# tencent-ailab/V-Express

Hardware: AMD Instinct MI355X
Metric: decoded frames/sec at 512x512, 25 DDIM steps (higher is better)
Workload: dtype bf16; 1 GPU; 512x512, 16 frames (1 window(s) of 16, overlap 4), 25 DDIM steps, CFG 3.5, random-init UNet3D + ReferenceNet banks + sd-vae-ft-mse decode; frames=16, windows=1, parallelism=window x CFG-half units over 1 GPU(s)

## Files before the change

### v-express_amd/csrc/vx_gemm.hip

```cpp
#include "vx_common.h"
#include "vx_gemm_common.h"
#include "../../include/vexpress_hip.h"

#include <stdio.h>
#include <stdlib.h>
#include <string.h>

namespace {

#ifdef VX_GEMM_ABLATE
#define ABL(bit) (((VX_GEMM_ABLATE) & (bit)) != 0)
#else
#define ABL(bit) false
#endif

struct RowInfo {
  int pix_base;
  int iy0, ix0;
};

template <typename T>
__device__ __forceinline__ T sel3(int i, T a, T b, T c) { return i == 0 ? a : (i == 1 ? b : c); }

__device__ __attribute__((aligned(16))) const uint4 g_zero16 = {0u, 0u, 0u, 0u};

template <int N>
__device__ __forceinline__ void wait_vmcnt() {
  asm volatile("s_waitcnt vmcnt(%0)" ::"n"(N) : "memory");
}

typedef int i32x8_t __attribute__((ext_vector_type(8)));
__device__ __forceinline__ f32x4_t mfma16_f8(const uint4& a_lo, const uint4& a_hi, const uint4& b_lo, const uint4& b_hi,
                                             f32x4_t c) {
  const i32x8_t a = {(int)a_lo.x, (int)a_lo.y, (int)a_lo.z, (int)a_lo.w, (int)a_hi.x, (int)a_hi.y, (int)a_hi.z, (int)a_hi.w};
  const i32x8_t b = {(int)b_lo.x, (int)b_lo.y, (int)b_lo.z, (int)b_lo.w, (int)b_hi.x, (int)b_hi.y, (int)b_hi.z, (int)b_hi.w};
  return __builtin_amdgcn_mfma_scale_f32_16x16x128_f8f6f4(a, b, c, 0, 0, 0, 0x7f7f7f7f, 0, 0x7f7f7f7f);
}

template <int BM, int BN, int WARPS_M, int WARPS_N, int STAGES, int EPI, bool FAST, bool F8 = false, bool LNF = false,
          bool GNS = false>
__global__ __launch_bounds__(64 * WARPS_M * WARPS_N, 2) void gemm_kernel(const vx_gemm_params p) {
  static_assert(!F8 || FAST, "fp8 operands use the FAST addressing only");
  static_assert(!GNS || (EPI == VX_EPI_STORE && !F8 && !LNF), "GroupNorm partial sums come from the plain STORE epilogue");
  static_assert(!LNF || (FAST && !F8), "a folded LayerNorm sits in front of a plain bf16 linear");
  constexpr int ES = F8 ? 1 : 2;
  constexpr int BKE = 128 / ES;
  constexpr int CE = 16 / ES;
  constexpr int NTHREADS = 64 * WARPS_M * WARPS_N;
  constexpr int RPP = NTHREADS / 8;
  constexpr int WM = BM / WARPS_M, WN = BN / WARPS_N;
  constexpr int MI = WM / 16, NI = WN / 16;
  constexpr int NJ = F8 ? (NI % 2 == 0 ? 2 : 1) : (NI <= 5 ? NI : NI / 2);
  constexpr int A_IT = BM / RPP, B_IT = BN / RPP;
  constexpr int G = A_IT + B_IT;
  constexpr int STAGE_BYTES = (BM + BN) * 128;
  static_assert(WM == 64, "every wave owns a 64-row slab");
  static_assert(BM % RPP == 0 && BN % RPP == 0, "tile rows must be a multiple of the staging pass");
  static_assert(NI % NJ == 0, "fragment grouping");
  static_assert(G * (STAGES - 2) < 64, "vmcnt is 6 bits");
  extern __shared__ __attribute__((aligned(16))) char smem[];

  const int tid = threadIdx.x;
  const int lane = tid & 63, wave = __builtin_amdgcn_readfirstlane(tid >> 6);
  const int wm = wave / WARPS_N, wn = wave % WARPS_N;
  const int n_tiles = (p.n + BN - 1) / BN;
  const int nsplit = (EPI == VX_EPI_STORE && p.splitk > 1) ? p.splitk : 1;
  const int lid0 = xcd_remap(blockIdx.x, gridDim.x);
  const int split = lid0 % nsplit, lid = lid0 / nsplit;
  const int tile_m = lid / n_tiles, tile_n = lid - tile_m * n_tiles;
  const int m0 = tile_m * BM, n0 = tile_n * BN;

  const bf16_t* __restrict__ A1 = (const bf16_t*)p.a;
  const bf16_t* __restrict__ A2 = (const bf16_t*)p.a2;
  const bf16_t* __restrict__ Wt = (const bf16_t*)p.w;
  const int cin = p.c1 + p.c2;
  const int c1 = p.c1;
  const int up = p.upsample;
  const int h_eff = p.h_in << up, w_eff = p.w_in << up;
  const int hw_out = p.h_out * p.w_out;
  const int w_in = p.w_in, kw = p.kw, kh = p.kh;
  const int lda1 = p.lda1, lda2 = p.lda2;
  const bf16_t* const zsrc = reinterpret_cast<const bf16_t*>(&g_zero16);

  const int r0 = tid >> 3;
  const int cc = (tid & 7) ^ ((r0 >> 1) & 7);
  uint32_t aoff1[A_IT], aoff2[A_IT], boff[B_IT];
  const int nk_total = (p.k + BKE - 1) / BKE;
  const int kt_begin = (int)((long)split * nk_total / nsplit), kt_end = (int)((long)(split + 1) * nk_total / nsplit);
  int s_kt = kt_begin, s_ci, s_kx, s_ky;
  {
    const int tap0 = (kt_begin * BKE) / cin;
    s_ci = kt_begin * BKE - tap0 * cin;
    s_ky = tap0 / kw;
    s_kx = tap0 - s_ky * kw;
  }
  RowInfo ri[A_IT];
  long wrow[B_IT];
// ... 153 lines not shown
#pragma unroll
        for (int i = 0; i < MI; ++i)
#pragma unroll
          for (int j = 0; j < NJ; ++j) {
            if (ABL(8)) {
              asm volatile("" ::"v"(bfr[j].x), "v"(af[i].x));
              continue;
            }
            acc[i][j0 + j] = mfma16(bfr[j], af[i], acc[i][j0 + j]);
          }
      }
    }
    }
    stage = stage + 1 == STAGES ? 0 : stage + 1;
    fill = fill + 1 == STAGES ? 0 : fill + 1;
  }

  const float* __restrict__ bias = p.bias;
  const int lrow = lane & 15, lq = lane >> 4;
  const int wrow0 = m0 + wm * WM, wcol0 = n0 + wn * WN;

  if constexpr (F8) {
    const float* __restrict__ asc = p.a_scale;
    const float* __restrict__ wsc = p.w_scale;
    float sa_[MI];
#pragma unroll
    for (int i = 0; i < MI; ++i) sa_[i] = asc[min(wrow0 + i * 16 + lrow, p.m - 1)];
#pragma unroll
    for (int j = 0; j < NI; ++j) {
      const float4 sw = *reinterpret_cast<const float4*>(wsc + min(wcol0 + j * 16 + lq * 4, p.n - 4));
#pragma unroll
      for (int i = 0; i < MI; ++i) {
        acc[i][j][0] *= sa_[i] * sw.x; acc[i][j][1] *= sa_[i] * sw.y;
        acc[i][j][2] *= sa_[i] * sw.z; acc[i][j][3] *= sa_[i] * sw.w;
      }
    }
  }

  if constexpr (LNF) {
    const float2* __restrict__ st = reinterpret_cast<const float2*>(p.ln_stats);
    const float* __restrict__ cs = p.ln_colsum;
#pragma unroll
    for (int i = 0; i < MI; ++i) {
      const float2 t = st[min(wrow0 + i * 16 + lrow, p.m - 1)];
#pragma unroll
      for (int j = 0; j < NI; ++j) {
        const float4 s4 = *reinterpret_cast<const float4*>(cs + min(wcol0 + j * 16 + lq * 4, p.n - 4));
        acc[i][j][0] = t.y * (acc[i][j][0] - t.x * s4.x); acc[i][j][1] = t.y * (acc[i][j][1] - t.x * s4.y);
        acc[i][j][2] = t.y * (acc[i][j][2] - t.x * s4.z); acc[i][j][3] = t.y * (acc[i][j][3] - t.x * s4.w);
      }
    }
  }

  if (EPI == VX_EPI_STORE && nsplit > 1) {
    float* ws = (float*)p.splitk_ws + (size_t)split * p.m * p.n;
#pragma unroll
    for (int i = 0; i < MI; ++i) {
      const int m = wrow0 + i * 16 + lrow;
#pragma unroll
      for (int j = 0; j < NI; ++j) {
        const int n = wcol0 + j * 16 + lq * 4;
        if (m < p.m && n < p.n)
          *reinterpret_cast<float4*>(ws + (size_t)m * p.n + n) =
              make_float4(acc[i][j][0], acc[i][j][1], acc[i][j][2], acc[i][j][3]);
      }
    }
    return;
  }
  if constexpr (EPI == VX_EPI_STORE) {
    const float* __restrict__ rowbias = p.rowbias;
    const bf16_t* __restrict__ resid = (const bf16_t*)p.residual;
    const bool do_silu = p.act == VX_ACT_SILU, do_gelu = p.act == VX_ACT_GELU;
    const bool out_is_f32 = p.out_f32 != 0;
    const float alpha = p.alpha;
    float gcs[GNS ? NI * 4 : 1], gcq[GNS ? NI * 4 : 1];
    if constexpr (GNS) {
#pragma unroll
      for (int c = 0; c < NI * 4; ++c) gcs[c] = gcq[c] = 0.f;
    }
#pragma unroll
    for (int j0 = 0; j0 < NI; j0 += NJ) {
      int ncol[NJ], nc[NJ];
      float4 bv[NJ];
#pragma unroll
      for (int j = 0; j < NJ; ++j) {
        ncol[j] = wcol0 + (j0 + j) * 16 + lq * 4;
        nc[j] = min(ncol[j], p.n - 4);
        bv[j] = make_float4(0.f, 0.f, 0.f, 0.f);
      }
      if (bias != nullptr && !ABL(2)) {
#pragma unroll
        for (int j = 0; j < NJ; ++j) bv[j] = *reinterpret_cast<const float4*>(bias + nc[j]);
      }
#pragma unroll
      for (int i = 0; i < MI; ++i) {
        const int m = wrow0 + i * 16 + lrow;
        const int mc = min(m, p.m - 1);
        uint2 rv[NJ];
        float4 rb[NJ];
#pragma unroll
        for (int j = 0; j < NJ; ++j) {
          rv[j] = make_uint2(0u, 0u);
          rb[j] = make_float4(0.f, 0.f, 0.f, 0.f);
        }
        if (resid != nullptr && !ABL(2)) {
          const bf16_t* rrow = resid + (size_t)mc * p.ldr;
#pragma unroll
          for (int j = 0; j < NJ; ++j) rv[j] = *reinterpret_cast<const uint2*>(rrow + nc[j]);
        }
        if (rowbias != nullptr && !ABL(2)) {
          const float* rbrow = rowbias + (size_t)(mc / p.rows_per_group) * p.rowbias_ld;
#pragma unroll
          for (int j = 0; j < NJ; ++j) rb[j] = *reinterpret_cast<const float4*>(rbrow + nc[j]);
        }
#pragma unroll
        for (int j = 0; j < NJ; ++j) {
          const f32x4_t a4 = acc[i][j0 + j];
          float v[4] = {a4[0] + bv[j].x + rb[j].x, a4[1] + bv[j].y + rb[j].y, a4[2] + bv[j].z + rb[j].z,
                        a4[3] + bv[j].w + rb[j].w};
          if (do_silu) {
#pragma unroll
            for (int e = 0; e < 4; ++e) v[e] = silu_f(v[e]);
          } else if (do_gelu) {
#pragma unroll
            for (int e = 0; e < 4; ++e) v[e] = gelu_f(v[e]);
          }
#pragma unroll
          for (int e = 0; e < 4; ++e) v[e] *= alpha;
          v[0] += e16_lo(rv[j].x); v[1] += e16_hi(rv[j].x);
          v[2] += e16_lo(rv[j].y); v[3] += e16_hi(rv[j].y);
          if constexpr (GNS) {
            const uint2 pk = make_uint2(pack_bf16x2(v[0], v[1]), pack_bf16x2(v[2], v[3]));
            *reinterpret_cast<uint2*>((bf16_t*)p.out + (size_t)m * p.ldc + ncol[j]) = pk;
            const float g[4] = {e16_lo(pk.x), e16_hi(pk.x),
                                e16_lo(pk.y), e16_hi(pk.y)};
#pragma unroll
            for (int e = 0; e < 4; ++e) {
              gcs[(j0 + j) * 4 + e] += g[e];
              gcq[(j0 + j) * 4 + e] = fmaf(g[e], g[e], gcq[(j0 + j) * 4 + e]);
            }
          } else if (ABL(1)) {
            asm volatile("" ::"v"(v[0]), "v"(v[1]), "v"(v[2]), "v"(v[3]));
          } else if (m < p.m && ncol[j] < p.n) {
            if (out_is_f32) {
              *reinterpret_cast<float4*>((float*)p.out + (size_t)m * p.ldc + ncol[j]) =
                  make_float4(v[0], v[1], v[2], v[3]);
            } else {
              *reinterpret_cast<uint2*>((bf16_t*)p.out + (size_t)m * p.ldc + ncol[j]) =
                  make_uint2(pack_bf16x2(v[0], v[1]), pack_bf16x2(v[2], v[3]));
            }
          }
        }
      }
    }
    if constexpr (GNS) {
#pragma unroll
      for (int c = 0; c < NI * 4; ++c) {
        gcs[c] = row16_sum(gcs[c]);
        gcq[c] = row16_sum(gcq[c]);
      }
      float2* scr = reinterpret_cast<float2*>(smem + STAGES * STAGE_BYTES) + wave * WN;
      if (lrow == 0) {
#pragma unroll
        for (int j = 0; j < NI; ++j)
#pragma unroll
          for (int e = 0; e < 4; ++e) scr[j * 16 + lq * 4 + e] = make_float2(gcs[j * 4 + e], gcq[j * 4 + e]);
      }
      asm volatile("s_waitcnt lgkmcnt(0)" ::: "memory");
      const int cg = p.n / p.gn_groups;
      if (lane < WN / cg) {
        float a = 0.f, b = 0.f;
        for (int c = 0; c < cg; ++c) {
          const float2 t = scr[lane * cg + c];
          a += t.x;
          b += t.y;
        }
        const int frame = wrow0 / p.gn_hw, slab = (wrow0 - frame * p.gn_hw) >> 6, slabs = p.gn_hw >> 6;
        const int g = wcol0 / cg + lane;
        reinterpret_cast<float2*>(p.gn_ws)[(size_t)(frame * slabs + slab) * p.gn_groups + g] = make_float2(a, b);
      }
    }
  } else if constexpr (EPI == VX_EPI_GEGLU) {
    static_assert(MI % 2 == 0, "GEGLU pairs row blocks");
// ... 106 lines not shown
        }
        __syncthreads();
      }
    }
  }
}

__global__ __launch_bounds__(256) void splitk_reduce_kernel(const vx_gemm_params p) {
  const int n4 = p.n >> 2;
  const long total = (long)p.m * n4;
  const float* __restrict__ ws = (const float*)p.splitk_ws;
  const size_t slab = (size_t)p.m * p.n;
  for (long idx = (long)blockIdx.x * 256 + threadIdx.x; idx < total; idx += (long)gridDim.x * 256) {
    const int m = (int)(idx / n4), n = (int)(idx - (long)m * n4) * 4;
    float4 a = *reinterpret_cast<const float4*>(ws + (size_t)m * p.n + n);
    for (int s = 1; s < p.splitk; ++s) {
      const float4 b = *reinterpret_cast<const float4*>(ws + s * slab + (size_t)m * p.n + n);
      a.x += b.x; a.y += b.y; a.z += b.z; a.w += b.w;
    }
    float v[4] = {a.x, a.y, a.z, a.w};
    if (p.bias != nullptr) {
      const float4 b = *reinterpret_cast<const float4*>(p.bias + n);
      v[0] += b.x; v[1] += b.y; v[2] += b.z; v[3] += b.w;
    }
    if (p.rowbias != nullptr) {
      const float4 b =
          *reinterpret_cast<const float4*>(p.rowbias + (size_t)(m / p.rows_per_group) * p.rowbias_ld + n);
      v[0] += b.x; v[1] += b.y; v[2] += b.z; v[3] += b.w;
    }
    if (p.act == VX_ACT_SILU) {
#pragma unroll
      for (int e = 0; e < 4; ++e) v[e] = silu_f(v[e]);
    } else if (p.act == VX_ACT_GELU) {
#pragma unroll
      for (int e = 0; e < 4; ++e) v[e] = gelu_f(v[e]);
    }
#pragma unroll
    for (int e = 0; e < 4; ++e) v[e] *= p.alpha;
    if (p.residual != nullptr) {
      const uint2 r2 = *reinterpret_cast<const uint2*>((const bf16_t*)p.residual + (size_t)m * p.ldr + n);
      v[0] += e16_lo(r2.x); v[1] += e16_hi(r2.x);
      v[2] += e16_lo(r2.y); v[3] += e16_hi(r2.y);
    }
    if (p.out_f32) {
      *reinterpret_cast<float4*>((float*)p.out + (size_t)m * p.ldc + n) = make_float4(v[0], v[1], v[2], v[3]);
    } else {
      *reinterpret_cast<uint2*>((bf16_t*)p.out + (size_t)m * p.ldc + n) =
          make_uint2(pack_bf16x2(v[0], v[1]), pack_bf16x2(v[2], v[3]));
    }
  }
}

template <int BM, int BN, int WARPS_M, int WARPS_N, int STAGES, int EPI, bool FAST, bool F8 = false, bool LNF = false,
          bool GNS = false>
int launch_impl(const vx_gemm_params& p, hipStream_t stream) {
  constexpr int stage_bytes = STAGES * (BM + BN) * 128;
  constexpr int epi_bytes = (EPI == VX_EPI_SPLIT) ? BN * (64 + 4) * 4 : 0;
  constexpr int gns_bytes = GNS ? WARPS_M * BN * 8 : 0;
  constexpr int smem = (stage_bytes > epi_bytes ? stage_bytes : epi_bytes) + gns_bytes;
  constexpr int nthreads = 64 * WARPS_M * WARPS_N;
  static bool attr_set = false;
  auto kern = gemm_kernel<BM, BN, WARPS_M, WARPS_N, STAGES, EPI, FAST, F8, LNF, GNS>;
  if (!attr_set) {
    hipError_t e = hipFuncSetAttribute((const void*)kern, hipFuncAttributeMaxDynamicSharedMemorySize, smem);
    if (e != hipSuccess) {
      vx_set_error("vx_gemm: hipFuncSetAttribute(%d B LDS) failed: %s", smem, hipGetErrorString(e));
      return VX_ERR_HIP;
    }
    attr_set = true;
  }
  const int nsplit = (EPI == VX_EPI_STORE && p.splitk > 1) ? p.splitk : 1;
  long tiles = (long)ceil_div(p.m, BM) * ceil_div(p.n, BN) * nsplit;
  static char sym[112] = "";
  if (!sym[0]) {
    auto b = [](bool v) { return v ? "true" : "false"; };
    snprintf(sym, sizeof(sym), "gemm_kernel<%d, %d, %d, %d, %d, %d, %s, %s, %s, %s>", BM, BN, WARPS_M, WARPS_N, STAGES, EPI,
             b(FAST), b(F8), b(LNF), b(GNS));
  }
  g_vx_last_kernel = sym;
  hipLaunchKernelGGL(kern, dim3((unsigned)tiles), dim3(nthreads), smem, stream, p);
  int rc = vx_check_launch("vx_gemm");
  if (rc != 0 || nsplit == 1) return rc;
  long work = ((long)p.m * (p.n >> 2) + 255) / 256;
  hipLaunchKernelGGL(splitk_reduce_kernel, dim3((unsigned)(work < 2048 ? work : 2048)), dim3(256), 0, stream, p);
  return vx_check_launch("vx_gemm(split-K reduce)");
}

bool fast_ok(const vx_gemm_params& p) { return vx_gemm_fast_ok(p); }
}
bool vx_gemm_fast_ok(const vx_gemm_params& p) {
  static int disabled = -1;
  if (disabled < 0) disabled = getenv("VX_GEMM_NOFAST") != nullptr;
  if (disabled) return false;
  const int cin = p.c1 + p.c2;
  const unsigned long long rows_in = (unsigned long long)p.nb * p.h_in * p.w_in;
  return p.pad == 0 && p.upsample == 0 && (cin % 64) == 0 && (p.c1 % 64) == 0 && (p.k % 64) == 0 &&
         rows_in * (unsigned long long)p.lda1 * 2ull < (1ull << 32) &&
         (p.c2 == 0 || rows_in * (unsigned long long)p.lda2 * 2ull < (1ull << 32)) &&
         (unsigned long long)p.n * p.k * 2ull < (1ull << 32) &&
         (p.h_out - 1) * p.stride + p.kh <= p.h_in && (p.w_out - 1) * p.stride + p.kw <= p.w_in;
}
namespace {

template <int BM, int BN, int WARPS_M, int WARPS_N, int STAGES, int EPI>
int launch(const vx_gemm_params& p, hipStream_t stream) {
  if (p.ln_stats != nullptr) {
    if (!fast_ok(p)) {
      vx_set_error("vx_gemm: a folded LayerNorm needs a plain linear (k %% 64 == 0, no padding / upsampling)");
      return VX_ERR_UNSUPPORTED;
    }
    return launch_impl<BM, BN, WARPS_M, WARPS_N, STAGES, EPI, true, false, true>(p, stream);
  }
  if (fast_ok(p)) return launch_impl<BM, BN, WARPS_M, WARPS_N, STAGES, EPI, true>(p, stream);
  return launch_impl<BM, BN, WARPS_M, WARPS_N, STAGES, EPI, false>(p, stream);
}

template <int BM, int BN, int WARPS_M, int WARPS_N, int STAGES>
int launch_gns(const vx_gemm_params& p, hipStream_t stream) {
  if (fast_ok(p)) return launch_impl<BM, BN, WARPS_M, WARPS_N, STAGES, VX_EPI_STORE, true, false, false, true>(p, stream);
  return launch_impl<BM, BN, WARPS_M, WARPS_N, STAGES, VX_EPI_STORE, false, false, false, true>(p, stream);
}

bool prefer160(int n) {
  int w160 = ceil_div(n, 160) * 160 - n, w128 = ceil_div(n, 128) * 128 - n;
  return w160 * 128 <= w128 * 160;
}

enum { CFG_AUTO = 0, CFG_BIG = 1, CFG_SMALL = 2 };
int forced_cfg() {
  static int v = -1;
  if (v < 0) {
    const char* e = getenv("VX_GEMM_TILE");
    v = CFG_AUTO;
    if (e && !strcmp(e, "big")) v = CFG_BIG;
    if (e && !strcmp(e, "small")) v = CFG_SMALL;
  }
  return v;
}
bool use_big(const vx_gemm_params& p) {
  if ((p.n % 320) != 0 || p.splitk > 1) return false;
  int f = forced_cfg();
  if (f == CFG_BIG) return true;
  if (f == CFG_SMALL) return false;
  long tiles = (long)ceil_div(p.m, 256) * (p.n / 320);
  return tiles >= 256;
}

bool use_small64(const vx_gemm_params& p) {
  static int on = -1;
  if (on < 0) {
    const char* e = getenv("VX_GEMM_SMALL64");
    on = !(e && !strcmp(e, "0"));
  }
  if (!on || !prefer160(p.n) || p.out_f32) return false;
  const long tiles128 = (long)ceil_div(p.m, 128) * ceil_div(p.n, 160) * (p.splitk > 1 ? p.splitk : 1);
  static long lim = -1;
  if (lim < 0) {
    const char* e = getenv("VX_GEMM_SMALL64_BELOW");
    lim = e ? atol(e) : 256;
  }
  return tiles128 < lim && fast_ok(p);
}

enum { T_256x32 = 0, T_BIG, T_SMALL64, T_128x160, T_128x128, T_128x320, T_256x256 };
bool use_256x256(const vx_gemm_params& p) {
  static int on = -1;
  if (on < 0) {
    const char* e = getenv("VX_GEMM_T256X256");
    on = !(e && !strcmp(e, "0"));
  }
  return on && (p.n % 256) == 0 && p.n <= 1024 && p.splitk <= 1 && !p.out_f32 && (long)ceil_div(p.m, 256) * (p.n / 256) >= 256;
}
bool use_128x320(const vx_gemm_params& p) {
// ... 2 lines not shown
    const char* e = getenv("VX_GEMM_T128X320");
    on = e && !strcmp(e, "1");
  }
  return on && (p.n % 320) == 0 && p.splitk <= 1 && !p.out_f32;
}
int store_tile(const vx_gemm_params& p, bool gn = false) {
  if (p.n <= 32) return T_256x32;
  if (gn && (p.n % 160) == 0) return use_small64(p) ? T_SMALL64 : T_128x160;
  if (use_big(p)) return T_BIG;
  if (use_small64(p)) return T_SMALL64;
  if (use_128x320(p)) return T_128x320;
  if (prefer160(p.n)) return T_128x160;
  if (use_256x256(p)) return T_256x256;
  return T_128x128;
}

}

extern "C" int vx_gemm_gn_slabs(const vx_gemm_params* pp) {
  const vx_gemm_params& p = *pp;
  if (p.epi != VX_EPI_STORE || p.a_fp8 || p.out_f32 || p.ln_stats != nullptr || p.row_stats_out != nullptr ||
      (p.splitk > 1 && p.ring_hint != 2) || p.w_group_rows != 0)
    return 0;
  if (p.gn_groups <= 0 || p.gn_hw <= 0 || p.n <= 0 || (p.n % p.gn_groups) != 0 || (p.m % p.gn_hw) != 0) return 0;
  if (vx_gemm_ring_eligible(p)) return vx_gemm_ring_gn_slabs(p);
  if (p.splitk > 1) return 0;
  const int cg = p.n / p.gn_groups;
  const int tile = store_tile(p, true);
  if (tile != T_SMALL64 && tile != T_128x160) return 0;
  static int st128 = -1;
  if (st128 < 0) {
    const char* e = getenv("VX_GEMM_STAGES128");
    st128 = e ? atoi(e) : 2;
  }
  if (tile == T_128x160 && st128 != 2) return 0;
  const int bm = tile == T_SMALL64 ? 64 : 128;
  if ((p.m % bm) != 0 || (p.n % 160) != 0 || (p.gn_hw % 64) != 0 || (80 % cg) != 0) return 0;
  return p.gn_hw / 64;
}

thread_local const char* g_vx_last_kernel = "";
extern "C" const char* vx_gemm_last_kernel(void) { return g_vx_last_kernel; }
extern "C" const char* vx_last_kernel(void) { return g_vx_last_kernel; }

extern "C" int vx_gemm_ring_coop_ok(const vx_gemm_params* pp) {
  vx_gemm_params q = *pp;
  q.ring_hint = 2;
  q.splitk = 2;
  if (q.splitk_ws == nullptr) q.splitk_ws = (void*)16;
  return vx_gemm_ring_eligible(q) ? 1 : 0;
}

extern "C" int64_t vx_gemm_splitk_ws_bytes(int m, int n, int splitk) {
  return splitk > 1 ? (int64_t)splitk * m * n * (int64_t)sizeof(float) : 0;
}

extern "C" const char* vx_gemm_config_name(const vx_gemm_params* pp) {
  const vx_gemm_params& p = *pp;
  const bool fast = fast_ok(p);
  const char* epi = p.epi == VX_EPI_STORE ? "STORE" : (p.epi == VX_EPI_GEGLU ? "GEGLU" : "SPLIT");
  const char* tile;
  if (p.a_fp8) {
    static thread_local char b8[96];
    if (p.epi == VX_EPI_STORE && vx_gemm_ring_eligible(p)) return "gemm_ring_kernel<256x320x128,8w,STORE,fast,fp8>";
    const bool big8 = (p.n % 320) == 0 && (long)ceil_div(p.m, 256) * (p.n / 320) >= 256;
    snprintf(b8, sizeof(b8), "gemm_kernel<%s,%s,fast,fp8>", big8 ? "256x320x128,8w" : "128x160x128,4w", epi);
    return b8;
  }
  if (vx_gemm_ring_eligible(p))
    return p.epi == VX_EPI_GEGLU ? "gemm_ring_kernel<256x320x64,8w,GEGLU,fast>"
                                 : (p.ring_hint == 2 ? "gemm_ring_kernel<256x320x64,8w,STORE,fast,coop2>"
                                                     : "gemm_ring_kernel<256x320x64,8w,STORE,fast>");
  if (p.epi == VX_EPI_STORE && p.n <= 32) tile = "256x32x64,4w";
  else if (use_big(p)) tile = "256x320x64,8w";
  else if (p.epi == VX_EPI_STORE && use_small64(p)) tile = "64x160x64,2w";
  else if (p.epi == VX_EPI_STORE && use_128x320(p)) tile = "128x320x64,8w";
  else if (p.epi == VX_EPI_STORE && !prefer160(p.n) && use_256x256(p)) tile = "256x256x64,8w";
  else if (p.epi != VX_EPI_GEGLU && prefer160(p.n)) tile = "128x160x64,4w";
  else tile = "128x128x64,4w";
  static thread_local char buf[96];
  if (p.splitk > 1)
    snprintf(buf, sizeof(buf), "gemm_kernel<%s,%s,%s,splitk%d>", tile, epi, fast ? "fast" : "gather", p.splitk);
  else
    snprintf(buf, sizeof(buf), "gemm_kernel<%s,%s,%s>", tile, epi, fast ? "fast" : "gather");
  return buf;
}

static int vx_gemm_dispatch(const vx_gemm_params& p, hipStream_t stream);

extern "C" int vx_gemm(const vx_gemm_params* pp, void* stream_) {
  const vx_gemm_params& p = *pp;
  hipStream_t stream = (hipStream_t)stream_;
  if (p.row_stats_out != nullptr)
    VX_REQUIRE(p.epi == VX_EPI_STORE && !p.out_f32 && p.row_stats_eps > 0.f && p.out != nullptr,
               "vx_gemm: row_stats_out needs the STORE epilogue into bf16 and row_stats_eps > 0");
  VX_REQUIRE(p.row_stats_parts == 0 || p.row_stats_parts == 1 || (p.row_stats_parts == 2 && p.n == 640),
             "vx_gemm: row_stats_parts=%d (0 / 1, or 2 with n == 640; n=%d)", p.row_stats_parts, p.n);
  if (p.ln_stats != nullptr && p.ln_stats_parts == 2) {
    if (p.k != 640 || !(p.ln_eps > 0.f) || !vx_gemm_ring_eligible(p)) {
      vx_set_error("vx_gemm: ln_stats_parts = 2 needs k == 640, ln_eps > 0 and a launch on the persistent kernel (k=%d m=%d "
                   "n=%d): convert with vx_row_stats_finalize", p.k, p.m, p.n);
      return VX_ERR_UNSUPPORTED;
    }
  } else {
    VX_REQUIRE(p.ln_stats_parts == 0 || p.ln_stats_parts == 1 || p.ln_stats == nullptr,
               "vx_gemm: ln_stats_parts=%d (0 / 1 / 2)", p.ln_stats_parts);
  }
  if (p.w_group_rows != 0)
    VX_REQUIRE(p.w_group_rows > 0 && (p.m % p.w_group_rows) == 0 && p.epi == VX_EPI_STORE && !p.a_fp8 && p.splitk <= 1,
               "vx_gemm: w_group_rows=%d must divide m=%d (STORE epilogue, no fp8 / split-K)", p.w_group_rows, p.m);
  if (p.gn_ws != nullptr && vx_gemm_gn_slabs(pp) <= 0) {
    vx_set_error("vx_gemm: this launch cannot produce GroupNorm partial sums (gn_ws set; vx_gemm_gn_slabs() == 0: m=%d "
                 "n=%d groups=%d hw=%d epi=%d splitk=%d)", p.m, p.n, p.gn_groups, p.gn_hw, p.epi, p.splitk);
    return VX_ERR_UNSUPPORTED;
  }
  const int rc = vx_gemm_dispatch(p, stream);
  if (rc != VX_OK || p.row_stats_out == nullptr) return rc;
  if (vx_gemm_ring_eligible(p) && vx_gemm_ring_writes_row_stats(p)) return rc;
  if (p.row_stats_parts == 2) return vx_row_stats_parts(p.out, p.ldc, p.m, p.n, p.row_stats_out, stream_);
  return vx_row_stats(p.out, p.ldc, p.m, p.n, p.row_stats_eps, p.row_stats_out, stream_);
}

static int vx_gemm_dispatch(const vx_gemm_params& p, hipStream_t stream) {
  VX_REQUIRE(p.a != nullptr && p.w != nullptr, "vx_gemm: null operand");
  VX_REQUIRE(p.m > 0 && p.n > 0 && p.k > 0, "vx_gemm: empty problem m=%d n=%d k=%d", p.m, p.n, p.k);
  VX_REQUIRE((p.c1 % 8) == 0 && (p.c2 % 8) == 0 && p.c1 > 0, "vx_gemm: channels must be multiples of 8 (c1=%d c2=%d)",
             p.c1, p.c2);
  VX_REQUIRE((p.c2 == 0) == (p.a2 == nullptr), "vx_gemm: a2/c2 mismatch");
  VX_REQUIRE(p.k == p.kh * p.kw * (p.c1 + p.c2), "vx_gemm: k=%d != kh*kw*(c1+c2)=%d", p.k,
             p.kh * p.kw * (p.c1 + p.c2));
  VX_REQUIRE(p.m == p.nb * p.h_out * p.w_out, "vx_gemm: m=%d != nb*h_out*w_out", p.m);
  VX_REQUIRE((p.n % 8) == 0, "vx_gemm: n=%d must be a multiple of 8", p.n);
  VX_REQUIRE((p.lda1 % 8) == 0 && (p.c2 == 0 || (p.lda2 % 8) == 0), "vx_gemm: lda must be a multiple of 8");
  VX_REQUIRE(p.upsample == 0 || p.upsample == 1, "vx_gemm: upsample must be 0/1");
  VX_REQUIRE(p.stride >= 1 && p.kh >= 1 && p.kw >= 1, "vx_gemm: bad conv geometry");
  VX_REQUIRE(p.ln_stats == nullptr || (p.ln_colsum != nullptr && p.splitk <= 1 && !p.a_fp8),
             "vx_gemm: a folded LayerNorm needs ln_colsum and excludes split-K / fp8 operands");
  VX_REQUIRE(p.splitk <= 1 || (p.epi == VX_EPI_STORE && p.splitk_ws != nullptr && p.splitk <= 16 &&
                               p.splitk <= (p.k + BK - 1) / BK),
             "vx_gemm: split-K needs the STORE epilogue, a workspace and splitk <= min(16, K/64)");
  if (p.a_fp8) {
    VX_REQUIRE(p.a_scale != nullptr && p.w_scale != nullptr, "vx_gemm(fp8): null scale table");
    VX_REQUIRE(p.kh == 1 && p.kw == 1 && p.stride == 1 && p.pad == 0 && p.upsample == 0 && p.a2 == nullptr &&
                   p.splitk <= 1 && p.h_out == p.h_in && p.w_out == p.w_in,
               "vx_gemm(fp8): plain linears only");
    VX_REQUIRE((p.k % 128) == 0 && (p.lda1 % 16) == 0 && p.c1 == p.k && (p.n % 4) == 0,
               "vx_gemm(fp8): k=%d must be a multiple of 128 (zero-padded), lda1=%d of 16", p.k, p.lda1);
    VX_REQUIRE((unsigned long long)p.m * p.lda1 < (1ull << 32) && (unsigned long long)p.n * p.k < (1ull << 32),
               "vx_gemm(fp8): operand spans 4 GiB");
    VX_REQUIRE(p.epi == VX_EPI_STORE || p.epi == VX_EPI_SPLIT, "vx_gemm(fp8): STORE / SPLIT epilogues only");
    const bool big = (p.n % 320) == 0 && (long)ceil_div(p.m, 256) * (p.n / 320) >= 256;
    if (p.epi == VX_EPI_STORE) {
      VX_REQUIRE(p.out != nullptr && (p.ldc % 8) == 0, "vx_gemm: STORE needs out and ldc%%8==0");
      VX_REQUIRE(p.residual == nullptr || (p.ldr % 8) == 0, "vx_gemm: ldr%%8");
      VX_REQUIRE(p.rowbias == nullptr || p.rows_per_group > 0, "vx_gemm: rows_per_group");
      if (vx_gemm_ring_eligible(p)) return vx_gemm_ring_launch(p, stream);
      if (big) return launch_impl<256, 320, 4, 2, 2, VX_EPI_STORE, true, true>(p, stream);
      return launch_impl<128, 160, 2, 2, 2, VX_EPI_STORE, true, true>(p, stream);
    }
  }
  if (p.epi == VX_EPI_STORE) {
    VX_REQUIRE(p.out != nullptr && (p.ldc % 8) == 0, "vx_gemm: STORE needs out and ldc%%8==0");
    VX_REQUIRE(p.residual == nullptr || (p.ldr % 8) == 0, "vx_gemm: ldr%%8");
    VX_REQUIRE(p.rowbias == nullptr || p.rows_per_group > 0, "vx_gemm: rows_per_group");
    if (p.ring_hint == 2 && (p.coop_epoch < 1 || p.coop_epoch >= (1 << 27))) {
      vx_set_error("vx_gemm: ring_hint = 2 needs 1 <= coop_epoch < 2^27 (the workspace's launch counter), got %d", p.coop_epoch);
      return VX_ERR_INVALID;
    }
    if (vx_gemm_ring_eligible(p)) return vx_gemm_ring_launch(p, stream);
    if (p.ring_hint == 2) {
      vx_set_error("vx_gemm: ring_hint = 2 (cooperative two-way K split on the persistent kernel) needs splitk == 2, a zeroed "
                   "workspace, m %% 256 == 0, n %% 320 == 0, an even number of 64-channel chunks and the plain STORE epilogue "
                   "(m=%d n=%d k=%d splitk=%d): ask vx_gemm_ring_coop_ok() first", p.m, p.n, p.k, p.splitk);
      return VX_ERR_UNSUPPORTED;
    }
    if (p.w_group_rows != 0) {
      vx_set_error("vx_gemm: per-row-group weights (w_group_rows=%d) need a launch the persistent 256 x 320 kernel "
                   "accepts (m %% 256, n %% 320, w_group_rows %% 256, plain addressing)", p.w_group_rows);
      return VX_ERR_UNSUPPORTED;
    }
    const int tile = store_tile(p, p.gn_ws != nullptr);
    if (p.gn_ws != nullptr) {
      if (tile == T_SMALL64) return launch_gns<64, 160, 1, 2, 3>(p, stream);
      return launch_gns<128, 160, 2, 2, 2>(p, stream);
    }
    if (tile == T_256x32) return launch<256, 32, 4, 1, 2, VX_EPI_STORE>(p, stream);
    if (tile == T_128x320) return launch<128, 320, 2, 4, 2, VX_EPI_STORE>(p, stream);
    if (tile == T_256x256) return launch<256, 256, 4, 2, 2, VX_EPI_STORE>(p, stream);
    if (tile == T_BIG) return launch<256, 320, 4, 2, 2, VX_EPI_STORE>(p, stream);
    if (tile == T_SMALL64) return launch<64, 160, 1, 2, 3, VX_EPI_STORE>(p, stream);
    if (tile == T_128x160) {
      static int st = -1;
      if (st < 0) {
        const char* e = getenv("VX_GEMM_STAGES128");
        st = e ? atoi(e) : 2;
      }
      if (st == 3) return launch<128, 160, 2, 2, 3, VX_EPI_STORE>(p, stream);
      if (st == 4) return launch<128, 160, 2, 2, 4, VX_EPI_STORE>(p, stream);
      return launch<128, 160, 2, 2, 2, VX_EPI_STORE>(p, stream);
    }
    return launch<128, 128, 2, 2, 2, VX_EPI_STORE>(p, stream);
  } else if (p.epi == VX_EPI_GEGLU) {
    VX_REQUIRE(p.out != nullptr && (p.n % 32) == 0 && (p.ldc % 8) == 0,
               "vx_gemm: GEGLU needs n%%32==0 (value/gate rows interleaved in blocks of 8)");
    if (vx_gemm_ring_eligible(p)) return vx_gemm_ring_launch(p, stream);
    if (use_big(p)) return launch<256, 320, 4, 2, 2, VX_EPI_GEGLU>(p, stream);
    return launch<128, 128, 2, 2, 2, VX_EPI_GEGLU>(p, stream);
  } else if (p.epi == VX_EPI_SPLIT) {
    VX_REQUIRE(p.n_parts >= 1 && p.n_parts <= 3 && p.part_cols > 0 && p.n == p.n_parts * p.part_cols,
               "vx_gemm: SPLIT n=%d != n_parts*part_cols", p.n);
    VX_REQUIRE((p.part_cols % 16) == 0, "vx_gemm: part_cols%%16 (a 16-column fragment must not straddle parts)");
    for (int i = 0; i < p.n_parts; ++i) {
      VX_REQUIRE(p.part_out[i] != nullptr, "vx_gemm: SPLIT part %d has no destination", i);
      if (p.part_kind[i] == VX_PART_VT)
        VX_REQUIRE(p.seq_len > 0 && p.head_dim > 0 && (p.part_cols % p.head_dim) == 0 && (p.vt_pitch % 8) == 0 &&
                       p.vt_pitch >= p.seq_len && (p.m % p.seq_len) == 0,
                   "vx_gemm: bad V^T geometry seq_len=%d head_dim=%d pitch=%d", p.seq_len, p.head_dim, p.vt_pitch);
      else
        VX_REQUIRE((p.part_ld[i] % 8) == 0, "vx_gemm: part_ld%%8");
    }
    if (p.a_fp8) {
      if ((p.n % 320) == 0 && (long)ceil_div(p.m, 256) * (p.n / 320) >= 256)
        return launch_impl<256, 320, 4, 2, 2, VX_EPI_SPLIT, true, true>(p, stream);
      return launch_impl<128, 160, 2, 2, 2, VX_EPI_SPLIT, true, true>(p, stream);
    }
    if (use_big(p)) return launch<256, 320, 4, 2, 2, VX_EPI_SPLIT>(p, stream);
    if (prefer160(p.n)) return launch<128, 160, 2, 2, 2, VX_EPI_SPLIT>(p, stream);
    return launch<128, 128, 2, 2, 2, VX_EPI_SPLIT>(p, stream);
  }
  vx_set_error("vx_gemm: unknown epilogue %d", p.epi);
  return VX_ERR_UNSUPPORTED;
}
```

### v-express_amd/csrc/vx_gemm_common.h

```cpp
#pragma once
#include "vx_common.h"
#include "../../include/vexpress_hip.h"

constexpr int BK = 64;

__device__ __forceinline__ int lds_off(int row, int chunk) { return row * 128 + ((chunk ^ ((row >> 1) & 7)) << 4); }

__device__ __forceinline__ uint32_t lds_addr_of(const void* shared_ptr) {
  return (uint32_t)(size_t)(__attribute__((address_space(3))) const char*)shared_ptr;
}
#ifndef VX_GLDS_MOD
#define VX_GLDS_MOD ""
#endif
__device__ __forceinline__ void glds16_s(const void* sbase, uint32_t voff, uint32_t lds_wave_addr) {
  asm volatile("s_mov_b32 m0, %0\n\ts_nop 0\n\tglobal_load_lds_dwordx4 %1, %2" VX_GLDS_MOD ::"s"(lds_wave_addr),
               "v"(voff), "s"(sbase)
               : "memory", "m0");
}
__device__ __forceinline__ void glds16_v(const void* vaddr, uint32_t lds_wave_addr) {
  asm volatile("s_mov_b32 m0, %0\n\ts_nop 0\n\tglobal_load_lds_dwordx4 %1, off" VX_GLDS_MOD ::"s"(lds_wave_addr),
               "v"(vaddr)
               : "memory", "m0");
}

#ifndef VX_XCD_ROWS
#define VX_XCD_ROWS 0
#endif

__device__ __forceinline__ int xcd_remap(int bid, int nblk) {
  const int q = nblk >> 3, r = nblk & 7, xcd = bid & 7, idx = bid >> 3;
  return (xcd < r ? xcd * (q + 1) : r * (q + 1) + (xcd - r) * q) + idx;
}


bool vx_gemm_fast_ok(const vx_gemm_params& p);
bool vx_gemm_ring_eligible(const vx_gemm_params& p);
int vx_gemm_ring_launch(const vx_gemm_params& p, hipStream_t stream);
bool vx_gemm_ring_writes_row_stats(const vx_gemm_params& p);
int vx_gemm_ring_gn_slabs(const vx_gemm_params& p);

template <int CTRL>
__device__ __forceinline__ float dpp_mov(float v) {
  return __builtin_bit_cast(float, __builtin_amdgcn_update_dpp(0, __builtin_bit_cast(int, v), CTRL, 0xf, 0xf, false));
}
__device__ __forceinline__ float row16_sum(float v) {
  v += dpp_mov<0x128>(v);
  v += dpp_mov<0x124>(v);
  v += dpp_mov<0x122>(v);
  v += dpp_mov<0x121>(v);
  return v;
}
```

### v-express_amd/ops.py

```python
import ctypes as C
import logging
import os

import torch

from . import lib as L

class _CurrentLib:

    def __getattr__(self, name):
        return getattr(L.current(), name)


_lib = _CurrentLib()


def __getattr__(name):
    if name == "BF16":
        return L.ELEM[0]
    raise AttributeError(name)


def _stream():
    return C.c_void_p(torch.cuda.current_stream().cuda_stream)
# ... 356 lines not shown

def quantize_fp8(x):
    return layernorm_fp8(x, None, None)


def _base_params(a, w, geom, a2=None):
    if isinstance(a, Fp8Rows):
        if not isinstance(w, Fp8Weight) or a2 is not None or geom is not None:
            raise TypeError("fp8 activations need an Fp8Weight and a plain linear (no conv geometry, one source)")
        if a.q.shape[1] != w.w8.shape[1]:
            raise ValueError(f"fp8 K mismatch: {a.q.shape[1]} vs {w.w8.shape[1]}")
        p = L.GemmParams()
        rows, kp = a.q.shape
        p.a, p.c1, p.lda1 = a.q.data_ptr(), kp, a.q.stride(0)
        p.a2, p.c2, p.lda2 = None, 0, 0
        geom = ConvGeom(1, rows, 1)
        p.nb, p.h_in, p.w_in = 1, rows, 1
        p.kh, p.kw, p.stride, p.pad, p.upsample = 1, 1, 1, 0, 0
        p.h_out, p.w_out = rows, 1
        p.w, p.n, p.k, p.m = w.w8.data_ptr(), w.w8.shape[0], kp, rows
        p.alpha = 1.0
        p.a_fp8, p.a_scale, p.w_scale = 1, a.scale.data_ptr(), w.scale.data_ptr()
        return p, geom
    _chk_bf16(a, "a")
    _chk_bf16(w, "w")
    p = L.GemmParams()
    lda1, rows = _row_stride(a)
    p.a, p.c1, p.lda1 = a.data_ptr(), a.shape[-1], lda1
    if a2 is not None:
        _chk_bf16(a2, "a2")
        lda2, rows2 = _row_stride(a2)
        if rows2 != rows:
            raise ValueError("a/a2 row mismatch")
        p.a2, p.c2, p.lda2 = a2.data_ptr(), a2.shape[-1], lda2
    else:
        p.a2, p.c2, p.lda2 = None, 0, 0
    if geom is None:
        geom = ConvGeom(1, rows, 1)
    if rows != geom.nb * geom.h_in * geom.w_in:
        raise ValueError(f"activation rows {rows} != nb*h*w {geom.nb * geom.h_in * geom.w_in}")
    p.nb, p.h_in, p.w_in = geom.nb, geom.h_in, geom.w_in
    p.kh, p.kw, p.stride, p.pad, p.upsample = geom.kh, geom.kw, geom.stride, geom.pad, geom.upsample
    p.h_out, p.w_out = geom.h_out, geom.w_out
    if not w.is_contiguous() or w.dim() != 2:
        raise ValueError("weight must be a contiguous [N, K] matrix")
    p.w, p.n, p.k, p.m = w.data_ptr(), w.shape[0], w.shape[1], geom.m
    p.alpha = 1.0
    return p, geom


_SPLITK_WS = {}
_SPLITK_ROWS = int(os.environ.get("VX_SPLITK_ROWS", "128"))
_SPLITK_TARGET = int(os.environ.get("VX_SPLITK_TARGET", "512"))
_FRAME_ROWS = [None]


def _stream_key(device):
    return torch.cuda.current_stream(device).cuda_stream if torch.device(device).type == "cuda" else 0


def clear_caches():
    _SPLITK_WS.clear()
    _PADDED.clear()
    _FP8_W.clear()
    _FF_PACKED.clear()
    _TB_PACKED.clear()
    _COOP_WS.clear()
    _COOP_OK.clear()


_ITEMS = [None]


class frame_rows:

    def __init__(self, hw, items=None):
        self.hw, self.items = hw, items

    def __enter__(self):
        self.prev = (_FRAME_ROWS[0], _ITEMS[0])
        _FRAME_ROWS[0], _ITEMS[0] = self.hw, self.items

    def __exit__(self, *a):
        _FRAME_ROWS[0], _ITEMS[0] = self.prev


RING_MODE = [int(os.environ.get("VX_GEMM_RING", "2")) if os.environ.get("VX_GEMM_RING", "2") in ("0", "1", "2") else 2]
FP8_RING = [os.environ.get("VX_FP8_RING") == "1"]


def _ring_off(k):
    return RING_MODE[0] == 0 or (RING_MODE[0] == 1 and k > 1280)


def _ring_hint(p):
    if _ring_off(p.k):
        return -1
    items = _ITEMS[0]
    if items is None or items <= 0 or p.m % items:
        return 0
    rows_item = p.m // items
    if rows_item % 256 or p.n % 320:
        return -1
    return 1 if (2 * rows_item // 256) * (p.n // 320) >= 192 else -1


QK_RING = [os.environ.get("VX_QK_RING", "1") != "0"]


def qk_on_ring(m, c):
    items = _ITEMS[0]
    if not QK_RING[0] or items is None or items <= 0 or m % items or (2 * c) % 320 or c % 64:
        return False
    rows_item = m // items
    return rows_item % 256 == 0 and (2 * rows_item // 256) * (2 * c // 320) >= 192 and not _ring_off(c)


def _splitk(p, geom, device, plain):
    nk = -(-p.k // 64)
    hw = _FRAME_ROWS[0] if plain else geom.h_out * geom.w_out
    if hw is None or hw > 64 or p.k < 2560:
        return
    tiles = (2048 // _SPLITK_ROWS) * -(-p.n // 160)
    s = min(-(-_SPLITK_TARGET // tiles), 8, nk // 4)
    if s < 2:
        return
    nbytes = int(_lib.vx_gemm_splitk_ws_bytes(p.m, p.n, s))
    key = (device, _stream_key(device), nbytes)
    ws = _SPLITK_WS.get(key)
    if ws is None:
        ws = _SPLITK_WS[key] = torch.empty(nbytes, device=device, dtype=torch.uint8)
    p.splitk, p.splitk_ws = s, ws.data_ptr()


RING_COOP = [os.environ.get("VX_RING_COOP", "1") != "0"]
COOP_MIN_K = [int(os.environ.get("VX_RING_COOP_MIN_K", "8192"))]
_COOP_WS = {}
_COOP_OK = {}
_COOP_EPOCH_MAX = (1 << 27) - 1


def _coop_signature(p, rows_item):
    return (rows_item, p.m, p.n, p.k, p.c1, p.c2, p.kh, p.kw, p.stride, p.lda1, p.lda2, p.ldc, p.ldr, bool(p.residual),
            bool(p.ln_stats), bool(p.row_stats_out), p.row_stats_parts, p.w_group_rows, bool(p.rowbias), p.rowbias_ld,
            p.rows_per_group, p.epi, p.out_f32, p.act)


def ring_coop_applies(p):
    items = _ITEMS[0]
    if items is None or items <= 0 or p.m % items or _ring_off(p.k):
        return False
    rows_item = p.m // items
    if rows_item % 256 or p.n % 320:
        return False
    tiles_pair = (2 * rows_item // 256) * (p.n // 320)
    if not 96 <= tiles_pair < 192:
        return False
    sig = _coop_signature(p, rows_item)
    lib_ok = _COOP_OK.get(sig)
    if lib_ok is None and RING_COOP[0] and p.k >= COOP_MIN_K[0]:
        lib_ok = _COOP_OK[sig] = bool(_lib.vx_gemm_ring_coop_ok(C.byref(p)))
    why = ("VX_RING_COOP=0" if not RING_COOP[0] else f"K below {COOP_MIN_K[0]}: break-even" if p.k < COOP_MIN_K[0] else
           "" if lib_ok else "the kernel's limits (epilogue / odd number of 64-channel chunks)")
    epi = ("+res" if p.residual else "") + ("+ln" if p.ln_stats else "") + ("+rowstats" if p.row_stats_out else "")
    return _note_path("gemm_too_few_tiles", (("rows_item", rows_item), ("n", p.n), ("k", p.k), ("chunks", (p.c1 + p.c2) // 64),
                                             ("epilogue", epi or "plain")), not why,
                      "persistent kernel, cooperative two-way K split" if not why else "128 x 160 tiles", why)


def _ring_coop(p, device):
    if not ring_coop_applies(p):
        return False
    nbytes = int(_lib.vx_gemm_splitk_ws_bytes(p.m, p.n, 2))
    key = (device, _stream_key(device), nbytes)
    ent = _COOP_WS.get(key)
    if ent is None or ent[1] >= _COOP_EPOCH_MAX:
        ent = _COOP_WS[key] = [torch.zeros(nbytes, device=device, dtype=torch.uint8), 0]
    ent[1] += 1
    p.splitk, p.splitk_ws, p.ring_hint, p.coop_epoch = 2, ent[0].data_ptr(), 2, ent[1]
    return True


def gemm(a, w, bias=None, *, geom=None, a2=None, residual=None, alpha=1.0, act=L.VX_ACT_NONE, rowbias=None,
         rows_per_group=0, out=None, out_f32=False, ln=None, stats_out=None, stats_eps=1e-5, w_group_rows=0, gn=None,
         a_pixel_offset=0):
# ... 697 lines not shown
```

Measured before the change: 14.18 frames/s.

## Fuse split-K reduction into GEMM via last-arriving-tile atomic counter

Split-K GEMMs now reduce their partial sums inside the same launch. Each tile writes its fp32 partial to the workspace and bumps a per-tile epoch-tagged atomic counter. The last split to arrive sums all slabs and runs the normal STORE epilogue. This removes the separate splitk_reduce kernel launch and its extra pass over the workspace, at the cost of atomics, an acquire fence, serial reduction work in the last CTA, and a zero-initialised counter region that carries epoch state between calls.

```diff
diff --git a/v-express_amd/csrc/vx_gemm.hip b/v-express_amd/csrc/vx_gemm.hip
--- a/v-express_amd/csrc/vx_gemm.hip
+++ b/v-express_amd/csrc/vx_gemm.hip
@@ -27,6 +27,20 @@
 template <int N>
 __device__ __forceinline__ void wait_vmcnt() {
   asm volatile("s_waitcnt vmcnt(%0)" ::"n"(N) : "memory");
+}
+
+typedef int sk_i32x4_t __attribute__((ext_vector_type(4)));
+__device__ __forceinline__ void sk_store16(__amdgpu_buffer_rsrc_t ws, uint32_t voff, uint32_t soff, const f32x4_t& v) {
+  __builtin_amdgcn_raw_buffer_store_b128(__builtin_bit_cast(sk_i32x4_t, v), ws, voff, soff, 16);
+}
+__device__ __forceinline__ f32x4_t sk_load16(__amdgpu_buffer_rsrc_t ws, uint32_t voff, uint32_t soff) {
+  return __builtin_bit_cast(f32x4_t, __builtin_amdgcn_raw_buffer_load_b128(ws, voff, soff, 16));
+}
+
+__device__ __forceinline__ float sk_mul_add(float v, float alpha, float r) {
+#pragma clang fp contract(off)
+  const float t = v * alpha;
+  return t + r;
 }
 
 typedef int i32x8_t __attribute__((ext_vector_type(8)));
@@ -38,11 +52,13 @@
 }
 
 template <int BM, int BN, int WARPS_M, int WARPS_N, int STAGES, int EPI, bool FAST, bool F8 = false, bool LNF = false,
-          bool GNS = false>
+          bool GNS = false, bool SK = false>
 __global__ __launch_bounds__(64 * WARPS_M * WARPS_N, 2) void gemm_kernel(const vx_gemm_params p) {
   static_assert(!F8 || FAST, "fp8 operands use the FAST addressing only");
   static_assert(!GNS || (EPI == VX_EPI_STORE && !F8 && !LNF), "GroupNorm partial sums come from the plain STORE epilogue");
   static_assert(!LNF || (FAST && !F8), "a folded LayerNorm sits in front of a plain bf16 linear");
+  static_assert(!SK || (EPI == VX_EPI_STORE && !F8 && !LNF && WARPS_M * 64 == BM && BM <= 128),
+                "in-launch split-K reduction: the plain STORE epilogue of the 64- and 128-row tiles");
   constexpr int ES = F8 ? 1 : 2;
   constexpr int BKE = 128 / ES;
   constexpr int CE = 16 / ES;
@@ -302,7 +318,7 @@
     }
   }
 
-  if (EPI == VX_EPI_STORE && nsplit > 1) {
+  if (!SK && EPI == VX_EPI_STORE && nsplit > 1) {
     float* ws = (float*)p.splitk_ws + (size_t)split * p.m * p.n;
 #pragma unroll
     for (int i = 0; i < MI; ++i) {
@@ -316,6 +332,62 @@
       }
     }
     return;
+  }
+  if constexpr (SK) {
+    const uint32_t slab_bytes = (uint32_t)p.m * (uint32_t)p.n * 4u;
+    const __amdgpu_buffer_rsrc_t wsr = __builtin_amdgcn_make_buffer_rsrc(
+        (char*)p.splitk_ws + VX_SPLITK_CTR_BYTES, 0, (int)(slab_bytes * (uint32_t)nsplit), 0x00020000);
+#pragma unroll
+    for (int i = 0; i < MI; ++i) {
+      const int m = wrow0 + i * 16 + lrow;
+#pragma unroll
+      for (int j = 0; j < NI; ++j) {
+        const int n = wcol0 + j * 16 + lq * 4;
+        if (m < p.m && n < p.n) sk_store16(wsr, ((uint32_t)m * (uint32_t)p.n + (uint32_t)n) * 4u, (uint32_t)split * slab_bytes, acc[i][j]);
+      }
+    }
+    asm volatile("s_waitcnt vmcnt(0)" ::: "memory");
+    __syncthreads();
+    int* const last_flag = reinterpret_cast<int*>(smem);
+    if (tid == 0) {
+      unsigned* cnt = reinterpret_cast<unsigned*>(p.splitk_ws) + lid;
+      const unsigned epoch = (unsigned)p.coop_epoch;
+      const unsigned before = __hip_atomic_fetch_max(cnt, epoch << 5, __ATOMIC_RELAXED, __HIP_MEMORY_SCOPE_AGENT);
+      const unsigned old =
+          __hip_atomic_fetch_add(cnt, before == 0xffffffffu ? 0u : 1u, __ATOMIC_RELAXED, __HIP_MEMORY_SCOPE_AGENT);
+      *last_flag = ((old >> 5) == epoch && (int)(old & 31u) + 1 == nsplit) ? 1 : 0;
+    }
+    __syncthreads();
+    if (*last_flag == 0) return;
+    __builtin_amdgcn_fence(__ATOMIC_ACQUIRE, "agent");
+    constexpr int MH = MI / 2;
+    for (int s = (split == 0 ? 1 : 0); s < nsplit; ++s) {
+      const uint32_t soff = (uint32_t)s * slab_bytes;
+#pragma unroll
+      for (int ih = 0; ih < MI; ih += MH) {
+        f32x4_t t[MH][NI];
+#pragma unroll
+        for (int i = 0; i < MH; ++i) {
+          const int m = min(wrow0 + (ih + i) * 16 + lrow, p.m - 1);
+#pragma unroll
+          for (int j = 0; j < NI; ++j) {
+            const int n = min(wcol0 + j * 16 + lq * 4, p.n - 4);
+            t[i][j] = sk_load16(wsr, ((uint32_t)m * (uint32_t)p.n + (uint32_t)n) * 4u, soff);
+          }
+        }
+#pragma unroll
+        for (int i = 0; i < MH; ++i)
+#pragma unroll
+          for (int j = 0; j < NI; ++j) {
+            if (s == 0) {
+              acc[ih + i][j] = t[i][j];
+            } else {
+              acc[ih + i][j][0] += t[i][j][0]; acc[ih + i][j][1] += t[i][j][1];
+              acc[ih + i][j][2] += t[i][j][2]; acc[ih + i][j][3] += t[i][j][3];
+            }
+          }
+      }
+    }
   }
   if constexpr (EPI == VX_EPI_STORE) {
     const float* __restrict__ rowbias = p.rowbias;
@@ -375,10 +447,15 @@
 #pragma unroll
             for (int e = 0; e < 4; ++e) v[e] = gelu_f(v[e]);
           }
-#pragma unroll
-          for (int e = 0; e < 4; ++e) v[e] *= alpha;
-          v[0] += e16_lo(rv[j].x); v[1] += e16_hi(rv[j].x);
-          v[2] += e16_lo(rv[j].y); v[3] += e16_hi(rv[j].y);
+          if constexpr (SK) {
+            v[0] = sk_mul_add(v[0], alpha, e16_lo(rv[j].x)); v[1] = sk_mul_add(v[1], alpha, e16_hi(rv[j].x));
+            v[2] = sk_mul_add(v[2], alpha, e16_lo(rv[j].y)); v[3] = sk_mul_add(v[3], alpha, e16_hi(rv[j].y));
+          } else {
+#pragma unroll
+            for (int e = 0; e < 4; ++e) v[e] *= alpha;
+            v[0] += e16_lo(rv[j].x); v[1] += e16_hi(rv[j].x);
+            v[2] += e16_lo(rv[j].y); v[3] += e16_hi(rv[j].y);
+          }
           if constexpr (GNS) {
             const uint2 pk = make_uint2(pack_bf16x2(v[0], v[1]), pack_bf16x2(v[2], v[3]));
             *reinterpret_cast<uint2*>((bf16_t*)p.out + (size_t)m * p.ldc + ncol[j]) = pk;
@@ -591,7 +668,7 @@
 }
 
 template <int BM, int BN, int WARPS_M, int WARPS_N, int STAGES, int EPI, bool FAST, bool F8 = false, bool LNF = false,
-          bool GNS = false>
+          bool GNS = false, bool SK = false>
 int launch_impl(const vx_gemm_params& p, hipStream_t stream) {
   constexpr int stage_bytes = STAGES * (BM + BN) * 128;
   constexpr int epi_bytes = (EPI == VX_EPI_SPLIT) ? BN * (64 + 4) * 4 : 0;
@@ -599,7 +676,7 @@
   constexpr int smem = (stage_bytes > epi_bytes ? stage_bytes : epi_bytes) + gns_bytes;
   constexpr int nthreads = 64 * WARPS_M * WARPS_N;
   static bool attr_set = false;
-  auto kern = gemm_kernel<BM, BN, WARPS_M, WARPS_N, STAGES, EPI, FAST, F8, LNF, GNS>;
+  auto kern = gemm_kernel<BM, BN, WARPS_M, WARPS_N, STAGES, EPI, FAST, F8, LNF, GNS, SK>;
   if (!attr_set) {
     hipError_t e = hipFuncSetAttribute((const void*)kern, hipFuncAttributeMaxDynamicSharedMemorySize, smem);
     if (e != hipSuccess) {
@@ -613,13 +690,13 @@
   static char sym[112] = "";
   if (!sym[0]) {
     auto b = [](bool v) { return v ? "true" : "false"; };
-    snprintf(sym, sizeof(sym), "gemm_kernel<%d, %d, %d, %d, %d, %d, %s, %s, %s, %s>", BM, BN, WARPS_M, WARPS_N, STAGES, EPI,
-             b(FAST), b(F8), b(LNF), b(GNS));
+    snprintf(sym, sizeof(sym), "gemm_kernel<%d, %d, %d, %d, %d, %d, %s, %s, %s, %s%s>", BM, BN, WARPS_M, WARPS_N, STAGES, EPI,
+             b(FAST), b(F8), b(LNF), b(GNS), SK ? ", true" : "");
   }
   g_vx_last_kernel = sym;
   hipLaunchKernelGGL(kern, dim3((unsigned)tiles), dim3(nthreads), smem, stream, p);
   int rc = vx_check_launch("vx_gemm");
-  if (rc != 0 || nsplit == 1) return rc;
+  if (rc != 0 || nsplit == 1 || SK) return rc;
   long work = ((long)p.m * (p.n >> 2) + 255) / 256;
   hipLaunchKernelGGL(splitk_reduce_kernel, dim3((unsigned)(work < 2048 ? work : 2048)), dim3(256), 0, stream, p);
   return vx_check_launch("vx_gemm(split-K reduce)");
@@ -658,6 +735,12 @@
 int launch_gns(const vx_gemm_params& p, hipStream_t stream) {
   if (fast_ok(p)) return launch_impl<BM, BN, WARPS_M, WARPS_N, STAGES, VX_EPI_STORE, true, false, false, true>(p, stream);
   return launch_impl<BM, BN, WARPS_M, WARPS_N, STAGES, VX_EPI_STORE, false, false, false, true>(p, stream);
+}
+
+template <int BM, int BN, int WARPS_M, int WARPS_N, int STAGES>
+int launch_sk(const vx_gemm_params& p, hipStream_t stream) {
+  if (fast_ok(p)) return launch_impl<BM, BN, WARPS_M, WARPS_N, STAGES, VX_EPI_STORE, true, false, false, false, true>(p, stream);
+  return launch_impl<BM, BN, WARPS_M, WARPS_N, STAGES, VX_EPI_STORE, false, false, false, false, true>(p, stream);
 }
 
 bool prefer160(int n) {
@@ -766,7 +849,7 @@
 }
 
 extern "C" int64_t vx_gemm_splitk_ws_bytes(int m, int n, int splitk) {
-  return splitk > 1 ? (int64_t)splitk * m * n * (int64_t)sizeof(float) : 0;
+  return splitk > 1 ? (int64_t)VX_SPLITK_CTR_BYTES + (int64_t)splitk * m * n * (int64_t)sizeof(float) : 0;
 }
 
 extern "C" const char* vx_gemm_config_name(const vx_gemm_params* pp) {
@@ -853,6 +936,13 @@
   VX_REQUIRE(p.splitk <= 1 || (p.epi == VX_EPI_STORE && p.splitk_ws != nullptr && p.splitk <= 16 &&
                                p.splitk <= (p.k + BK - 1) / BK),
              "vx_gemm: split-K needs the STORE epilogue, a workspace and splitk <= min(16, K/64)");
+  if (p.splitk > 1 && p.ring_hint != 2 && p.coop_epoch != 0) {
+    VX_REQUIRE(p.coop_epoch >= 1 && p.coop_epoch < (1 << 27), "vx_gemm: split-K coop_epoch=%d outside 1 .. 2^27 - 1", p.coop_epoch);
+    VX_REQUIRE((long long)p.splitk * p.m * p.n * 4 < (1ll << 31) &&
+                   (long long)ceil_div(p.m, 64) * ceil_div(p.n, 32) * 4 <= VX_SPLITK_CTR_BYTES,
+               "vx_gemm: split-K with coop_epoch (in-launch reduction) needs splitk * m * n * 4 < 2 GiB and at most %d tiles "
+               "(m=%d n=%d splitk=%d): use coop_epoch = 0", VX_SPLITK_CTR_BYTES / 4, p.m, p.n, p.splitk);
+  }
   if (p.a_fp8) {
     VX_REQUIRE(p.a_scale != nullptr && p.w_scale != nullptr, "vx_gemm(fp8): null scale table");
     VX_REQUIRE(p.kh == 1 && p.kw == 1 && p.stride == 1 && p.pad == 0 && p.upsample == 0 && p.a2 == nullptr &&
@@ -897,6 +987,13 @@
     if (p.gn_ws != nullptr) {
       if (tile == T_SMALL64) return launch_gns<64, 160, 1, 2, 3>(p, stream);
       return launch_gns<128, 160, 2, 2, 2>(p, stream);
+    }
+    if (p.splitk > 1 && p.coop_epoch > 0) {
+      if (tile == T_SMALL64) return launch_sk<64, 160, 1, 2, 3>(p, stream);
+      if (tile == T_128x160) return launch_sk<128, 160, 2, 2, 2>(p, stream);
+      if (tile == T_128x128) return launch_sk<128, 128, 2, 2, 2>(p, stream);
+      vx_set_error("vx_gemm: no in-launch split-K reduction for n <= 32 (n=%d): use coop_epoch = 0 (two launches)", p.n);
+      return VX_ERR_UNSUPPORTED;
     }
     if (tile == T_256x32) return launch<256, 32, 4, 1, 2, VX_EPI_STORE>(p, stream);
     if (tile == T_128x320) return launch<128, 320, 2, 4, 2, VX_EPI_STORE>(p, stream);
diff --git a/v-express_amd/csrc/vx_gemm_common.h b/v-express_amd/csrc/vx_gemm_common.h
--- a/v-express_amd/csrc/vx_gemm_common.h
+++ b/v-express_amd/csrc/vx_gemm_common.h
@@ -2,6 +2,7 @@
 #include "vx_common.h"
 #include "../../include/vexpress_hip.h"
 
+constexpr int VX_SPLITK_CTR_BYTES = 64 * 1024;
 constexpr int BK = 64;
 
 __device__ __forceinline__ int lds_off(int row, int chunk) { return row * 128 + ((chunk ^ ((row >> 1) & 7)) << 4); }
diff --git a/v-express_amd/ops.py b/v-express_amd/ops.py
--- a/v-express_amd/ops.py
+++ b/v-express_amd/ops.py
@@ -432,6 +432,8 @@
 _SPLITK_WS = {}
 _SPLITK_ROWS = int(os.environ.get("VX_SPLITK_ROWS", "128"))
 _SPLITK_TARGET = int(os.environ.get("VX_SPLITK_TARGET", "512"))
+SPLITK_INKERNEL = [os.environ.get("VX_SPLITK_INKERNEL", "1") != "0"]
+_SPLITK_MAX_TILES = 16384
 _FRAME_ROWS = [None]
 
 
@@ -507,10 +509,13 @@
         return
     nbytes = int(_lib.vx_gemm_splitk_ws_bytes(p.m, p.n, s))
     key = (device, _stream_key(device), nbytes)
-    ws = _SPLITK_WS.get(key)
-    if ws is None:
-        ws = _SPLITK_WS[key] = torch.empty(nbytes, device=device, dtype=torch.uint8)
-    p.splitk, p.splitk_ws = s, ws.data_ptr()
+    ent = _SPLITK_WS.get(key)
+    if ent is None or ent[1] >= _COOP_EPOCH_MAX:
+        ent = _SPLITK_WS[key] = [torch.zeros(nbytes, device=device, dtype=torch.uint8), 0]
+    p.splitk, p.splitk_ws = s, ent[0].data_ptr()
+    if SPLITK_INKERNEL[0] and s * p.m * p.n * 4 < (1 << 31) and -(-p.m // 64) * -(-p.n // 32) <= _SPLITK_MAX_TILES:
+        ent[1] += 1
+        p.coop_epoch = ent[1]
 
 
 RING_COOP = [os.environ.get("VX_RING_COOP", "1") != "0"]
```

Result: no change. 14.05 frames/s (-0.9%).
